# bupt-cist/vqa-playground-pytorch

Measured on AMD Instinct MI355X. Metric: VQA samples/sec (fwd+bwd), CoR2 batch 512, 36x2048 regions, higher is better.
Workload: dtype f32

## Files before the change

### vqa_playground_pytorch_amd/csrc/attention_logits.hip

```cpp
#include <cstdlib>
#include <type_traits>

#include "gemm_f32_rt.hpp"

namespace vqa {

constexpr int kAlMaxG = 8;
constexpr int kAlThreads = 256;
constexpr int kAlWaves = kAlThreads / 64;

template <typename T>
struct AlVec;
template <>
struct AlVec<float> {
  static constexpr int VEC = 2, P = 4;
  static __device__ __forceinline__ void ldb(rt::rsrc_t r, uint32_t voff, uint32_t soff, float (&v)[2]) {
    const auto t = __builtin_bit_cast(float2, __builtin_amdgcn_raw_buffer_load_b64(r, (int)voff, (int)soff, 0));
    v[0] = t.x;
    v[1] = t.y;
  }
  static __device__ __forceinline__ void stb(rt::rsrc_t r, uint32_t voff, uint32_t soff, const float (&v)[2]) {
    typedef unsigned int u32x2 __attribute__((ext_vector_type(2)));
    __builtin_amdgcn_raw_buffer_store_b64(u32x2{__float_as_uint(v[0]), __float_as_uint(v[1])}, r, (int)voff, (int)soff, 0);
  }
  static __device__ __forceinline__ void ld(const float* p, float (&v)[2]) {
    const float2 t = ld2(p);
    v[0] = t.x;
    v[1] = t.y;
  }
  static __device__ __forceinline__ void st(float* p, const float (&v)[2]) { st2(p, make_float2(v[0], v[1])); }
};
template <>
struct AlVec<bf16> {
  static constexpr int VEC = 4, P = 2;
  static __device__ __forceinline__ void ldb(rt::rsrc_t r, uint32_t voff, uint32_t soff, float (&v)[4]) {
    const auto w = __builtin_bit_cast(uint2, __builtin_amdgcn_raw_buffer_load_b64(r, (int)voff, (int)soff, 0));
    v[0] = bf16_lo(w.x);
    v[1] = bf16_hi(w.x);
    v[2] = bf16_lo(w.y);
    v[3] = bf16_hi(w.y);
  }
  static __device__ __forceinline__ void stb(rt::rsrc_t r, uint32_t voff, uint32_t soff, const float (&v)[4]) {
    typedef unsigned int u32x2 __attribute__((ext_vector_type(2)));
    __builtin_amdgcn_raw_buffer_store_b64(u32x2{pack_bf16(v[0], v[1]), pack_bf16(v[2], v[3])}, r, (int)voff, (int)soff, 0);
  }
  static __device__ __forceinline__ void ld(const bf16* p, float (&v)[4]) {
    const float4 t = ld4(p);
    v[0] = t.x;
    v[1] = t.y;
    v[2] = t.z;
    v[3] = t.w;
  }
  static __device__ __forceinline__ void st(bf16* p, const float (&v)[4]) { st4(p, make_float4(v[0], v[1], v[2], v[3])); }
};

struct AlMask {
  uint32_t key, p8;
  float scale;
};
__device__ __forceinline__ AlMask al_mask(const DropCfg& dc) { return AlMask{dc.p8 > 0 ? drop_key(dc) : 0u, dc.p8, dc.scale}; }
template <int MODE, int VEC>
__device__ __forceinline__ void al_keep(uint32_t e, const AlMask& mk, float (&s)[VEC]) {
#pragma unroll
  for (int j = 0; j < VEC; j += 2) {
    if constexpr (MODE == 0) {
      s[j] = 1.f, s[j + 1] = 1.f;
    } else if constexpr (MODE == 1) {
      const uint32_t w = mask_word32((e + j) >> 5, mk.key) >> ((e + j) & 31u);
      s[j] = (w & 1u) != 0u ? 2.f : 0.f;
      s[j + 1] = (w & 2u) != 0u ? 2.f : 0.f;
    } else {
      const uint32_t w = mask_word32((e + j) >> 2, mk.key) >> (8 * ((e + j) & 3));
      s[j] = (w & 255u) >= mk.p8 ? mk.scale : 0.f;
      s[j + 1] = ((w >> 8) & 255u) >= mk.p8 ? mk.scale : 0.f;
    }
  }
}
template <int G, int P, int VEC>
__device__ __forceinline__ void al_load_weights(const float* __restrict__ w, int K, int lane, float (&wr)[G][P][VEC]) {
#pragma unroll
  for (int g = 0; g < G; ++g)
#pragma unroll
    for (int p = 0; p < P; ++p)
#pragma unroll
      for (int j = 0; j < VEC; ++j) {
        const int k = (p * 64 + lane) * VEC + j;
        const float t = w[(size_t)g * K + min(k, K - 1)];
        wr[g][p][j] = k < K ? t : 0.f;
      }
}

constexpr int kAlRows = 8;

template <typename T, int G, int MODE>
__global__ __launch_bounds__(kAlThreads, 2) void attention_logits_fwd_kernel(const T* __restrict__ x, int ldx,
                                                                          const float* __restrict__ w,
                                                                          const float* __restrict__ bias,
                                                                          float* __restrict__ logits, int M, int K,
                                                                          DropCfg dc) {
  using V = AlVec<T>;
  constexpr int VEC = V::VEC, P = V::P, RB = kAlRows;
  constexpr bool BUTTERFLY = (RB * G) % 16 == 0 && 16 % G == 0;
  const int lane = threadIdx.x & 63;
  const int wave = blockIdx.x * kAlWaves + __builtin_amdgcn_readfirstlane(threadIdx.x >> 6), nwaves = gridDim.x * kAlWaves;
  float xv[RB][P][VEC];
  const int m_first = wave * RB;
  const rt::rsrc_t Xb = rt::make_rsrc(x, (size_t)M * ldx * sizeof(T));
  uint32_t voff[P];
#pragma unroll
  for (int p = 0; p < P; ++p) voff[p] = (uint32_t)min((p * 64 + lane) * VEC, ldx - VEC) * (uint32_t)sizeof(T);
  auto load_rows = [&](int m0) {
#pragma unroll
    for (int r = 0; r < RB; ++r) {
      const uint32_t soff = (uint32_t)min(m0 + r, M - 1) * (uint32_t)ldx * (uint32_t)sizeof(T);
#pragma unroll
      for (int p = 0; p < P; ++p) V::ldb(Xb, voff[p], soff, xv[r][p]);
    }
  };
  if (m_first < M) load_rows(m_first);
  float wr[G][P][VEC];
  al_load_weights<G, P, VEC>(w, K, lane, wr);
  const float bias_l = bias[(lane & 15) % G];
  const AlMask mk = al_mask(dc);
  for (int m0 = m_first; m0 < M; m0 += nwaves * RB) {
    if (m0 != m_first) load_rows(m0);
    float acc[RB][G];
    {
#pragma unroll
      for (int r = 0; r < RB; ++r) {
        const int m = min(m0 + r, M - 1);
#pragma unroll
        for (int g = 0; g < G; ++g) acc[r][g] = 0.f;
#pragma unroll
        for (int p = 0; p < P; ++p) {
          const int k = (p * 64 + lane) * VEC;
          float s[VEC];
          al_keep<MODE, VEC>((uint32_t)m * (uint32_t)K + (uint32_t)k, mk, s);
#pragma unroll
          for (int j = 0; j < VEC; ++j) {
            const float xs = xv[r][p][j] * s[j];
#pragma unroll
            for (int g = 0; g < G; ++g) acc[r][g] = fmaf(wr[g][p][j], xs, acc[r][g]);
          }
        }
        __builtin_amdgcn_sched_barrier(0);
      }
    }
    if constexpr (BUTTERFLY) {
      constexpr int RPB = 16 / G;
#pragma unroll
      for (int q = 0; q < RB / RPB; ++q) {
        float val[16];
#pragma unroll
        for (int i = 0; i < 16; ++i) val[i] = acc[q * RPB + i / G][i % G];
        const float t = rows_sum(row_reduce_scatter16(val, lane));
        const int m = m0 + q * RPB + (lane & 15) / G;
        if (lane < 16 && m < M) logits[(size_t)m * G + (lane & 15) % G] = t + bias_l;
      }
    } else {
#pragma unroll
      for (int r = 0; r < RB; ++r)
#pragma unroll
        for (int g = 0; g < G; ++g) {
          const float t = wave_sum(acc[r][g]);
          if (lane == 0 && m0 + r < M) logits[(size_t)(m0 + r) * G + g] = t + bias[g];
        }
    }
  }
}

constexpr int kAlBwdRows = 6;

template <typename T, int G, int MODE>
__global__ __launch_bounds__(kAlThreads, 2) void attention_logits_bwd_kernel(const T* __restrict__ x, int ldx,
                                                                          const float* __restrict__ w,
                                                                          const float* __restrict__ d_logits,
                                                                          T* __restrict__ d_x, float* __restrict__ part,
                                                                          float* __restrict__ partb, int M, int K,
                                                                          DropCfg dc) {
  using V = AlVec<T>;
  constexpr int VEC = V::VEC, P = V::P, RB = kAlBwdRows, KPAD = 64 * VEC * P;
  __shared__ float red_s[kAlWaves - 1][G][KPAD];
  __shared__ float redb_s[kAlWaves][G];
  const int lane = threadIdx.x & 63, wv = __builtin_amdgcn_readfirstlane(threadIdx.x >> 6);
  const int wave = blockIdx.x * kAlWaves + wv, nwaves = gridDim.x * kAlWaves;
  float wr[G][P][VEC], dw[G][P][VEC], db[G];
  al_load_weights<G, P, VEC>(w, K, lane, wr);
#pragma unroll
  for (int g = 0; g < G; ++g) {
    db[g] = 0.f;
#pragma unroll
    for (int p = 0; p < P; ++p)
#pragma unroll
      for (int j = 0; j < VEC; ++j) dw[g][p][j] = 0.f;
  }
  const AlMask mk = al_mask(dc);
  const rt::rsrc_t Xb = rt::make_rsrc(x, (size_t)M * ldx * sizeof(T));
  const rt::rsrc_t Db = rt::make_rsrc(d_x != nullptr ? d_x : const_cast<T*>(x), (size_t)M * ldx * sizeof(T));
  uint32_t voff[P];
#pragma unroll
  for (int p = 0; p < P; ++p) voff[p] = (uint32_t)min((p * 64 + lane) * VEC, ldx - VEC) * (uint32_t)sizeof(T);
  for (int m0 = wave * RB; m0 < M; m0 += nwaves * RB) {
    float xv[RB][P][VEC];
#pragma unroll
    for (int r = 0; r < RB; ++r) {
      const uint32_t soff = (uint32_t)min(m0 + r, M - 1) * (uint32_t)ldx * (uint32_t)sizeof(T);
#pragma unroll
      for (int p = 0; p < P; ++p) V::ldb(Xb, voff[p], soff, xv[r][p]);
    }
    float dl[RB][G];
#pragma unroll
    for (int r = 0; r < RB; ++r)
#pragma unroll
      for (int g = 0; g < G; ++g) {
        const float t = d_logits[(size_t)min(m0 + r, M - 1) * G + g];
        dl[r][g] = m0 + r < M ? t : 0.f;
      }
    {
#pragma unroll
      for (int r = 0; r < RB; ++r) {
        const int m = m0 + r;
#pragma unroll
        for (int g = 0; g < G; ++g) db[g] += dl[r][g];
#pragma unroll
        for (int p = 0; p < P; ++p) {
          const int k = (p * 64 + lane) * VEC;
          float s[VEC], o[VEC];
          al_keep<MODE, VEC>((uint32_t)min(m, M - 1) * (uint32_t)K + (uint32_t)k, mk, s);
#pragma unroll
          for (int j = 0; j < VEC; ++j) {
            const float xs = xv[r][p][j] * s[j];
            float t = 0.f;
#pragma unroll
            for (int g = 0; g < G; ++g) {
              dw[g][p][j] = fmaf(dl[r][g], xs, dw[g][p][j]);
              t = fmaf(dl[r][g], wr[g][p][j], t);
            }
            o[j] = t * s[j];
          }
          if (d_x != nullptr && m < M && k < ldx)
            V::stb(Db, (uint32_t)k * (uint32_t)sizeof(T), (uint32_t)m * (uint32_t)ldx * (uint32_t)sizeof(T), o);
        }
        __builtin_amdgcn_sched_barrier(0);
      }
    }
  }
  if (wv > 0) {
#pragma unroll
    for (int g = 0; g < G; ++g)
#pragma unroll
      for (int p = 0; p < P; ++p)
#pragma unroll
        for (int j = 0; j < VEC; ++j) red_s[wv - 1][g][(p * 64 + lane) * VEC + j] = dw[g][p][j];
  }
  if (lane == 0) {
#pragma unroll
    for (int g = 0; g < G; ++g) redb_s[wv][g] = db[g];
  }
  __syncthreads();
  if (wv == 0) {
#pragma unroll
    for (int g = 0; g < G; ++g)
#pragma unroll
      for (int p = 0; p < P; ++p)
#pragma unroll
        for (int j = 0; j < VEC; ++j) {
          const int k = (p * 64 + lane) * VEC + j;
          float t = dw[g][p][j];
#pragma unroll
          for (int q = 0; q < kAlWaves - 1; ++q) t += red_s[q][g][k];
          part[((size_t)blockIdx.x * G + g) * KPAD + k] = t;
        }
    if (lane < G) partb[(size_t)blockIdx.x * G + lane] = redb_s[0][lane] + redb_s[1][lane] + redb_s[2][lane] + redb_s[3][lane];
  }
}

__global__ __launch_bounds__(256) void attention_logits_finish_kernel(const float* __restrict__ part,
                                                                      const float* __restrict__ partb,
                                                                      float* __restrict__ d_w, float* __restrict__ d_bias,
                                                                      int K, int G, int KPAD, int nblocks) {
  __shared__ float red_s[16][17];
  const int c = threadIdx.x & 15, slice = threadIdx.x >> 4;
  const int e = blockIdx.x * 16 + c;
  const bool is_w = e < G * K, is_b = !is_w && e < G * K + G;
  const float* src = partb;
  size_t stride = (size_t)G, off = 0;
  if (is_w) {
    src = part;
    stride = (size_t)G * KPAD;
    off = (size_t)(e / K) * KPAD + (e % K);
  } else if (is_b) {
    off = (size_t)(e - G * K);
  }
  float a = 0.f;
  if (is_w || is_b) {
    for (int b0 = slice; b0 < nblocks; b0 += 256) {
      float t[16];
#pragma unroll
      for (int i = 0; i < 16; ++i) {
        const int b = b0 + 16 * i;
        t[i] = b < nblocks ? src[(size_t)b * stride + off] : 0.f;
      }
#pragma unroll
      for (int i = 0; i < 16; ++i) a += t[i];
    }
  }
  red_s[slice][c] = a;
  __syncthreads();
  if (slice == 0) {
    float t = 0.f;
#pragma unroll
    for (int q = 0; q < 16; ++q) t += red_s[q][c];
    if (is_w) d_w[e] = t;
    if (is_b) d_bias[e - G * K] = t;
  }
}

static int al_blocks(int M) {
  int b = (M + kAlBwdRows * kAlWaves - 1) / (kAlBwdRows * kAlWaves);
  if (b > 512) b = 512;
  if (b < 1) b = 1;
  return b;
}

template <typename T>
static int al_check(const char* who, const T* x, int ldx, int M, int K, int G, float p_drop) {
  using V = AlVec<T>;
  VQA_REQUIRE(M > 0 && K > 0 && G > 0, VQA_E_BADARG, "%s: bad sizes M=%d K=%d G=%d", who, M, K, G);
  VQA_REQUIRE(p_drop >= 0.f && p_drop < 1.f, VQA_E_BADARG, "%s: p_drop=%f outside [0,1)", who, (double)p_drop);
  VQA_REQUIRE(G <= kAlMaxG && K <= 64 * V::VEC * V::P && K % 2 == 0 && ldx >= K && ldx % V::VEC == 0 &&
                  aligned(x, V::VEC * sizeof(T)) && (size_t)M * ldx * sizeof(T) < (1ull << 32),
              VQA_E_UNSUPPORTED, "%s: needs G <= 8, even K <= %d, ldx %% %d == 0, aligned x, M*ldx*sizeof < 4 GiB (K=%d ldx=%d G=%d)", who,
              64 * V::VEC * V::P, V::VEC, K, ldx, G);
  return VQA_OK;
}

#define VQA_AL_SWITCH_G(G, CALL)      \
  switch (G) {                        \
    case 1: { CALL(1); } break;       \
    case 2: { CALL(2); } break;       \
    case 3: { CALL(3); } break;       \
    case 4: { CALL(4); } break;       \
    case 5: { CALL(5); } break;       \
    case 6: { CALL(6); } break;       \
    case 7: { CALL(7); } break;       \
    default: { CALL(8); } break;      \
  }

template <typename T>
static int al_fwd_impl(const char* who, const T* x, int ldx, const float* w, const float* bias, float* logits, float p_drop,
                       uint64_t seed, const uint64_t* seed_ptr, int M, int K, int G, vqa_stream_t stream) {
  VQA_REQUIRE(x && w && bias && logits, VQA_E_BADARG, "%s: null pointer", who);
  int rc = al_check(who, x, ldx, M, K, G, p_drop);
  if (rc != VQA_OK) return rc;
  hipStream_t s = static_cast<hipStream_t>(stream);
  const DropCfg dc = make_drop(p_drop, seed, seed_ptr);
  int blocks = (M + kAlRows * kAlWaves - 1) / (kAlRows * kAlWaves);
  if (blocks > 2048) blocks = 2048;
  const int mode = dc.p8 == 0 ? 0 : (dc.p8 == kDropHalf ? 1 : 2);
#define CALL_M(G_, MODE_) \
  VQA_LAUNCH((attention_logits_fwd_kernel<T, G_, MODE_>), dim3(blocks), dim3(kAlThreads), 0, s, x, ldx, w, bias, logits, M, K, dc)
#define CALL(G_)                       \
  if (mode == 0) CALL_M(G_, 0);        \
  else if (mode == 1) CALL_M(G_, 1);   \
  else CALL_M(G_, 2)
  VQA_AL_SWITCH_G(G, CALL);
#undef CALL
#undef CALL_M
  return check_launch(who);
}

template <typename T>
static size_t al_ws_bytes(int M, int G) {
  using V = AlVec<T>;
  return (size_t)al_blocks(M) * G * (64 * V::VEC * V::P + 1) * sizeof(float);
}

template <typename T>
static int al_bwd_impl(const char* who, const T* x, int ldx, const float* w, const float* d_logits, T* d_x, float* d_w,
                       float* d_bias, void* workspace, size_t workspace_bytes, float p_drop, uint64_t seed,
                       const uint64_t* seed_ptr, int M, int K, int G, vqa_stream_t stream) {
  using V = AlVec<T>;
  VQA_REQUIRE(x && w && d_logits && d_w && d_bias && workspace, VQA_E_BADARG, "%s: null pointer", who);
  int rc = al_check(who, x, ldx, M, K, G, p_drop);
  if (rc != VQA_OK) return rc;
  VQA_REQUIRE(d_x == nullptr || aligned(d_x, V::VEC * sizeof(T)), VQA_E_UNSUPPORTED, "%s: d_x is not aligned", who);
  VQA_REQUIRE(workspace_bytes >= al_ws_bytes<T>(M, G), VQA_E_BADARG, "%s: workspace of %zu B is too small", who, workspace_bytes);
  hipStream_t s = static_cast<hipStream_t>(stream);
  const DropCfg dc = make_drop(p_drop, seed, seed_ptr);
  const int blocks = al_blocks(M);
  constexpr int KPAD = 64 * V::VEC * V::P;
  float* part = static_cast<float*>(workspace);
  float* partb = part + (size_t)blocks * G * KPAD;
  const int mode = dc.p8 == 0 ? 0 : (dc.p8 == kDropHalf ? 1 : 2);
#define CALL_M(G_, MODE_)                                                                                                        \
  VQA_LAUNCH((attention_logits_bwd_kernel<T, G_, MODE_>), dim3(blocks), dim3(kAlThreads), 0, s, x, ldx, w, d_logits, d_x, \
                     part, partb, M, K, dc)
#define CALL(G_)                       \
  if (mode == 0) CALL_M(G_, 0);        \
  else if (mode == 1) CALL_M(G_, 1);   \
  else CALL_M(G_, 2)
  VQA_AL_SWITCH_G(G, CALL);
#undef CALL
#undef CALL_M
  VQA_LAUNCH(attention_logits_finish_kernel, dim3((G * K + G + 15) / 16), dim3(256), 0, s, part, partb, d_w, d_bias, K,
                     G, KPAD, blocks);
  return check_launch(who);
}

}

using namespace vqa;

extern "C" int vqa_attention_logits_fwd(const float* x, int ldx, const float* w, const float* bias, float* logits,
                                        float p_drop, uint64_t seed, const uint64_t* seed_ptr, int M, int K, int G,
                                        vqa_stream_t stream) {
  return al_fwd_impl<float>("attention_logits_fwd", x, ldx, w, bias, logits, p_drop, seed, seed_ptr, M, K, G, stream);
}
extern "C" int vqa_attention_logits_fwd_bf16(const vqa_bf16_t* x, int ldx, const float* w, const float* bias, float* logits,
                                             float p_drop, uint64_t seed, const uint64_t* seed_ptr, int M, int K, int G,
                                             vqa_stream_t stream) {
  return al_fwd_impl<bf16>("attention_logits_fwd_bf16", reinterpret_cast<const bf16*>(x), ldx, w, bias, logits, p_drop, seed,
                           seed_ptr, M, K, G, stream);
}
extern "C" size_t vqa_attention_logits_bwd_workspace_bytes(int M, int K, int G) {
  if (M <= 0 || K <= 0 || G <= 0 || G > kAlMaxG) return 0;
  return al_ws_bytes<float>(M, G) > al_ws_bytes<bf16>(M, G) ? al_ws_bytes<float>(M, G) : al_ws_bytes<bf16>(M, G);
}
extern "C" int vqa_attention_logits_bwd(const float* x, int ldx, const float* w, const float* d_logits, float* d_x,
                                        float* d_w, float* d_bias, void* workspace, size_t workspace_bytes, float p_drop,
                                        uint64_t seed, const uint64_t* seed_ptr, int M, int K, int G, vqa_stream_t stream) {
  return al_bwd_impl<float>("attention_logits_bwd", x, ldx, w, d_logits, d_x, d_w, d_bias, workspace, workspace_bytes, p_drop,
                            seed, seed_ptr, M, K, G, stream);
}
extern "C" int vqa_attention_logits_bwd_bf16(const vqa_bf16_t* x, int ldx, const float* w, const float* d_logits,
                                             vqa_bf16_t* d_x, float* d_w, float* d_bias, void* workspace,
                                             size_t workspace_bytes, float p_drop, uint64_t seed, const uint64_t* seed_ptr,
                                             int M, int K, int G, vqa_stream_t stream) {
  return al_bwd_impl<bf16>("attention_logits_bwd_bf16", reinterpret_cast<const bf16*>(x), ldx, w, d_logits,
                           reinterpret_cast<bf16*>(d_x), d_w, d_bias, workspace, workspace_bytes, p_drop, seed, seed_ptr, M, K,
                           G, stream);
}
```

Measured before the change: 260,800.

## Triple-buffer row loads and widen vector accesses in attention logits kernels

Result: no change. 261,200, median of 4 (+0.2%).

```diff
diff --git a/vqa_playground_pytorch_amd/csrc/attention_logits.hip b/vqa_playground_pytorch_amd/csrc/attention_logits.hip
--- a/vqa_playground_pytorch_amd/csrc/attention_logits.hip
+++ b/vqa_playground_pytorch_amd/csrc/attention_logits.hip
@@ -6,91 +6,106 @@
 namespace vqa {
 
 constexpr int kAlMaxG = 8;
-constexpr int kAlThreads = 256;
-constexpr int kAlWaves = kAlThreads / 64;
+constexpr int kAlCus = 256;
+constexpr int kAlKpad = 512;
+constexpr int kAlThreads = 256, kAlWaves = kAlThreads / 64;
+constexpr int kAlBwdThreads = 512, kAlBwdWaves = kAlBwdThreads / 64;
+static_assert(kAlBwdThreads == kAlKpad, "the backward kernel's LDS pass gives every thread one column");
 
 template <typename T>
 struct AlVec;
 template <>
 struct AlVec<float> {
-  static constexpr int VEC = 2, P = 4;
-  static __device__ __forceinline__ void ldb(rt::rsrc_t r, uint32_t voff, uint32_t soff, float (&v)[2]) {
-    const auto t = __builtin_bit_cast(float2, __builtin_amdgcn_raw_buffer_load_b64(r, (int)voff, (int)soff, 0));
-    v[0] = t.x;
-    v[1] = t.y;
-  }
-  static __device__ __forceinline__ void stb(rt::rsrc_t r, uint32_t voff, uint32_t soff, const float (&v)[2]) {
-    typedef unsigned int u32x2 __attribute__((ext_vector_type(2)));
-    __builtin_amdgcn_raw_buffer_store_b64(u32x2{__float_as_uint(v[0]), __float_as_uint(v[1])}, r, (int)voff, (int)soff, 0);
-  }
-  static __device__ __forceinline__ void ld(const float* p, float (&v)[2]) {
-    const float2 t = ld2(p);
-    v[0] = t.x;
-    v[1] = t.y;
-  }
-  static __device__ __forceinline__ void st(float* p, const float (&v)[2]) { st2(p, make_float2(v[0], v[1])); }
+  static constexpr int VEC = 4, P = 2, HALF = 2;
+  static __device__ __forceinline__ void unpack(rt::u32x4 r, float (&v)[4]) {
+#pragma unroll
+    for (int j = 0; j < 4; ++j) v[j] = __uint_as_float(r[j]);
+  }
+  static __device__ __forceinline__ rt::u32x4 pack(const float (&v)[4]) {
+    return rt::u32x4{__float_as_uint(v[0]), __float_as_uint(v[1]), __float_as_uint(v[2]), __float_as_uint(v[3])};
+  }
 };
 template <>
 struct AlVec<bf16> {
-  static constexpr int VEC = 4, P = 2;
-  static __device__ __forceinline__ void ldb(rt::rsrc_t r, uint32_t voff, uint32_t soff, float (&v)[4]) {
-    const auto w = __builtin_bit_cast(uint2, __builtin_amdgcn_raw_buffer_load_b64(r, (int)voff, (int)soff, 0));
-    v[0] = bf16_lo(w.x);
-    v[1] = bf16_hi(w.x);
-    v[2] = bf16_lo(w.y);
-    v[3] = bf16_hi(w.y);
-  }
-  static __device__ __forceinline__ void stb(rt::rsrc_t r, uint32_t voff, uint32_t soff, const float (&v)[4]) {
-    typedef unsigned int u32x2 __attribute__((ext_vector_type(2)));
-    __builtin_amdgcn_raw_buffer_store_b64(u32x2{pack_bf16(v[0], v[1]), pack_bf16(v[2], v[3])}, r, (int)voff, (int)soff, 0);
-  }
-  static __device__ __forceinline__ void ld(const bf16* p, float (&v)[4]) {
-    const float4 t = ld4(p);
-    v[0] = t.x;
-    v[1] = t.y;
-    v[2] = t.z;
-    v[3] = t.w;
-  }
-  static __device__ __forceinline__ void st(bf16* p, const float (&v)[4]) { st4(p, make_float4(v[0], v[1], v[2], v[3])); }
+  static constexpr int VEC = 8, P = 1, HALF = 4;
+  static __device__ __forceinline__ void unpack(rt::u32x4 r, float (&v)[8]) {
+#pragma unroll
+    for (int j = 0; j < 4; ++j) v[2 * j] = bf16_lo(r[j]), v[2 * j + 1] = bf16_hi(r[j]);
+  }
+  static __device__ __forceinline__ rt::u32x4 pack(const float (&v)[8]) {
+    return rt::u32x4{pack_bf16(v[0], v[1]), pack_bf16(v[2], v[3]), pack_bf16(v[4], v[5]), pack_bf16(v[6], v[7])};
+  }
 };
+__device__ __forceinline__ rt::u32x4 al_ldb(rt::rsrc_t r, uint32_t voff, uint32_t soff) {
+  return __builtin_amdgcn_raw_buffer_load_b128(r, (int)voff, (int)soff, 0);
+}
+__device__ __forceinline__ void al_stb(rt::rsrc_t r, uint32_t voff, uint32_t soff, rt::u32x4 v) {
+  __builtin_amdgcn_raw_buffer_store_b128(v, r, (int)voff, (int)soff, 0);
+}
+__device__ __forceinline__ void al_stb_half(rt::rsrc_t r, uint32_t voff, uint32_t soff, rt::u32x4 v) {
+  typedef unsigned int u32x2 __attribute__((ext_vector_type(2)));
+  __builtin_amdgcn_raw_buffer_store_b64(u32x2{v[0], v[1]}, r, (int)voff, (int)soff, 0);
+}
 
 struct AlMask {
   uint32_t key, p8;
   float scale;
 };
 __device__ __forceinline__ AlMask al_mask(const DropCfg& dc) { return AlMask{dc.p8 > 0 ? drop_key(dc) : 0u, dc.p8, dc.scale}; }
+template <int MODE>
+__device__ __forceinline__ uint32_t al_row_words(uint32_t e_row, int lane, const AlMask& mk) {
+  if constexpr (MODE == 1) return mask_word32((e_row >> 5) + (uint32_t)lane, mk.key);
+  return 0u;
+}
 template <int MODE, int VEC>
-__device__ __forceinline__ void al_keep(uint32_t e, const AlMask& mk, float (&s)[VEC]) {
-#pragma unroll
-  for (int j = 0; j < VEC; j += 2) {
-    if constexpr (MODE == 0) {
-      s[j] = 1.f, s[j + 1] = 1.f;
-    } else if constexpr (MODE == 1) {
-      const uint32_t w = mask_word32((e + j) >> 5, mk.key) >> ((e + j) & 31u);
-      s[j] = (w & 1u) != 0u ? 2.f : 0.f;
-      s[j + 1] = (w & 2u) != 0u ? 2.f : 0.f;
-    } else {
-      const uint32_t w = mask_word32((e + j) >> 2, mk.key) >> (8 * ((e + j) & 3));
-      s[j] = (w & 255u) >= mk.p8 ? mk.scale : 0.f;
-      s[j + 1] = ((w >> 8) & 255u) >= mk.p8 ? mk.scale : 0.f;
+__device__ __forceinline__ void al_keep(uint32_t e_row, uint32_t col, uint32_t row_words, const AlMask& mk, float (&s)[VEC]) {
+  if constexpr (MODE == 0) {
+#pragma unroll
+    for (int j = 0; j < VEC; ++j) s[j] = 1.f;
+  } else if constexpr (MODE == 1) {
+    const uint32_t bp = (e_row & 31u) + col;
+    const int at = (int)((bp >> 5) << 2);
+    const uint32_t w0 = (uint32_t)__builtin_amdgcn_ds_bpermute(at, (int)row_words);
+    const uint32_t w1 = (uint32_t)__builtin_amdgcn_ds_bpermute(at + 4, (int)row_words);
+    const uint32_t bits = __builtin_amdgcn_alignbit(w1, w0, bp & 31u);
+#pragma unroll
+    for (int j = 0; j < VEC; ++j) s[j] = __uint_as_float((0u - ((bits >> j) & 1u)) & 0x40000000u);
+  } else {
+    const uint32_t wi = (e_row + col) >> 2, shift = 8u * (e_row & 3u);
+    uint32_t hw[VEC / 4 + 1];
+#pragma unroll
+    for (int i = 0; i < VEC / 4; ++i) hw[i] = mask_word32(wi + (uint32_t)i, mk.key);
+    hw[VEC / 4] = shift != 0u ? mask_word32(wi + (uint32_t)(VEC / 4), mk.key) : 0u;
+#pragma unroll
+    for (int i = 0; i < VEC / 4; ++i) {
+      const uint32_t v = __builtin_amdgcn_alignbit(hw[i + 1], hw[i], shift);
+#pragma unroll
+      for (int b = 0; b < 4; ++b) s[4 * i + b] = ((v >> (8 * b)) & 255u) >= mk.p8 ? mk.scale : 0.f;
     }
   }
 }
 template <int G, int P, int VEC>
 __device__ __forceinline__ void al_load_weights(const float* __restrict__ w, int K, int lane, float (&wr)[G][P][VEC]) {
+  const rt::rsrc_t Wb = rt::make_rsrc(w, (size_t)G * K * sizeof(float));
 #pragma unroll
   for (int g = 0; g < G; ++g)
 #pragma unroll
     for (int p = 0; p < P; ++p)
 #pragma unroll
-      for (int j = 0; j < VEC; ++j) {
+      for (int j = 0; j < VEC; j += 4) {
         const int k = (p * 64 + lane) * VEC + j;
-        const float t = w[(size_t)g * K + min(k, K - 1)];
-        wr[g][p][j] = k < K ? t : 0.f;
+        const rt::u32x4 t = al_ldb(Wb, (uint32_t)k * (uint32_t)sizeof(float), (uint32_t)(g * K) * (uint32_t)sizeof(float));
+#pragma unroll
+        for (int i = 0; i < 4; ++i) wr[g][p][j + i] = k + i < K ? __uint_as_float(t[i]) : 0.f;
       }
 }
 
-constexpr int kAlRows = 8;
+constexpr int kAlRows = 3;
+
+__device__ __forceinline__ void al_share(int wave, int nwaves, int M, int& lo, int& hi) {
+  lo = (int)((long long)wave * M / nwaves);
+  hi = (int)((long long)(wave + 1) * M / nwaves);
+}
 
 template <typename T, int G, int MODE>
 __global__ __launch_bounds__(kAlThreads, 2) void attention_logits_fwd_kernel(const T* __restrict__ x, int ldx,
@@ -100,62 +115,66 @@
                                                                           DropCfg dc) {
   using V = AlVec<T>;
   constexpr int VEC = V::VEC, P = V::P, RB = kAlRows;
-  constexpr bool BUTTERFLY = (RB * G) % 16 == 0 && 16 % G == 0;
+  constexpr bool BUTTERFLY = 16 % G == 0;
   const int lane = threadIdx.x & 63;
   const int wave = blockIdx.x * kAlWaves + __builtin_amdgcn_readfirstlane(threadIdx.x >> 6), nwaves = gridDim.x * kAlWaves;
-  float xv[RB][P][VEC];
-  const int m_first = wave * RB;
+  int m_lo, m_hi;
+  al_share(wave, nwaves, M, m_lo, m_hi);
+  if (m_lo >= m_hi) return;
   const rt::rsrc_t Xb = rt::make_rsrc(x, (size_t)M * ldx * sizeof(T));
-  uint32_t voff[P];
-#pragma unroll
-  for (int p = 0; p < P; ++p) voff[p] = (uint32_t)min((p * 64 + lane) * VEC, ldx - VEC) * (uint32_t)sizeof(T);
-  auto load_rows = [&](int m0) {
+  uint32_t col[P];
+#pragma unroll
+  for (int p = 0; p < P; ++p) col[p] = (uint32_t)((p * 64 + lane) * VEC);
+  auto load_rows = [&](rt::u32x4 (&buf)[RB][P], int m0) {
 #pragma unroll
     for (int r = 0; r < RB; ++r) {
-      const uint32_t soff = (uint32_t)min(m0 + r, M - 1) * (uint32_t)ldx * (uint32_t)sizeof(T);
-#pragma unroll
-      for (int p = 0; p < P; ++p) V::ldb(Xb, voff[p], soff, xv[r][p]);
+      const uint32_t soff = (uint32_t)min(m0 + r, m_hi - 1) * (uint32_t)ldx * (uint32_t)sizeof(T);
+#pragma unroll
+      for (int p = 0; p < P; ++p) buf[r][p] = al_ldb(Xb, col[p] * (uint32_t)sizeof(T), soff);
     }
   };
-  if (m_first < M) load_rows(m_first);
+  rt::u32x4 b0[RB][P], b1[RB][P], b2[RB][P];
+  load_rows(b0, m_lo);
+  load_rows(b1, m_lo + RB);
   float wr[G][P][VEC];
   al_load_weights<G, P, VEC>(w, K, lane, wr);
   const float bias_l = bias[(lane & 15) % G];
   const AlMask mk = al_mask(dc);
-  for (int m0 = m_first; m0 < M; m0 += nwaves * RB) {
-    if (m0 != m_first) load_rows(m0);
+  auto work = [&](const rt::u32x4 (&buf)[RB][P], int m0) {
     float acc[RB][G];
-    {
-#pragma unroll
-      for (int r = 0; r < RB; ++r) {
-        const int m = min(m0 + r, M - 1);
-#pragma unroll
-        for (int g = 0; g < G; ++g) acc[r][g] = 0.f;
+#pragma unroll
+    for (int r = 0; r < RB; ++r) {
+#pragma unroll
+      for (int g = 0; g < G; ++g) acc[r][g] = 0.f;
+      if (m0 + r < m_hi) {
+        const uint32_t e_row = (uint32_t)(m0 + r) * (uint32_t)K;
+        const uint32_t words = al_row_words<MODE>(e_row, lane, mk);
 #pragma unroll
         for (int p = 0; p < P; ++p) {
-          const int k = (p * 64 + lane) * VEC;
-          float s[VEC];
-          al_keep<MODE, VEC>((uint32_t)m * (uint32_t)K + (uint32_t)k, mk, s);
+          float xv[VEC], s[VEC];
+          V::unpack(buf[r][p], xv);
+          al_keep<MODE, VEC>(e_row, col[p], words, mk, s);
 #pragma unroll
           for (int j = 0; j < VEC; ++j) {
-            const float xs = xv[r][p][j] * s[j];
+            const float xk = (int)col[p] + j < K ? xv[j] : 0.f;
+            const float xs = MODE == 0 ? xk : xk * s[j];
 #pragma unroll
             for (int g = 0; g < G; ++g) acc[r][g] = fmaf(wr[g][p][j], xs, acc[r][g]);
           }
         }
-        __builtin_amdgcn_sched_barrier(0);
       }
+      __builtin_amdgcn_sched_barrier(0);
     }
     if constexpr (BUTTERFLY) {
       constexpr int RPB = 16 / G;
 #pragma unroll
-      for (int q = 0; q < RB / RPB; ++q) {
+      for (int q = 0; q * RPB < RB; ++q) {
         float val[16];
 #pragma unroll
-        for (int i = 0; i < 16; ++i) val[i] = acc[q * RPB + i / G][i % G];
+        for (int i = 0; i < 16; ++i) val[i] = q * RPB + i / G < RB ? acc[min(q * RPB + i / G, RB - 1)][i % G] : 0.f;
         const float t = rows_sum(row_reduce_scatter16(val, lane));
-        const int m = m0 + q * RPB + (lane & 15) / G;
-        if (lane < 16 && m < M) logits[(size_t)m * G + (lane & 15) % G] = t + bias_l;
+        const int r = q * RPB + (lane & 15) / G;
+        if (lane < 16 && r < RB && m0 + r < m_hi) logits[(size_t)(m0 + r) * G + (lane & 15) % G] = t + bias_l;
       }
     } else {
 #pragma unroll
@@ -163,115 +182,148 @@
 #pragma unroll
         for (int g = 0; g < G; ++g) {
           const float t = wave_sum(acc[r][g]);
-          if (lane == 0 && m0 + r < M) logits[(size_t)(m0 + r) * G + g] = t + bias[g];
+          if (lane == 0 && m0 + r < m_hi) logits[(size_t)(m0 + r) * G + g] = t + bias[g];
         }
     }
-  }
-}
-
-constexpr int kAlBwdRows = 6;
+  };
+  for (int m0 = m_lo;; m0 += 3 * RB) {
+    load_rows(b2, m0 + 2 * RB);
+    work(b0, m0);
+    if (m0 + RB >= m_hi) break;
+    load_rows(b0, m0 + 3 * RB);
+    work(b1, m0 + RB);
+    if (m0 + 2 * RB >= m_hi) break;
+    load_rows(b1, m0 + 4 * RB);
+    work(b2, m0 + 2 * RB);
+    if (m0 + 3 * RB >= m_hi) break;
+  }
+}
 
 template <typename T, int G, int MODE>
-__global__ __launch_bounds__(kAlThreads, 2) void attention_logits_bwd_kernel(const T* __restrict__ x, int ldx,
-                                                                          const float* __restrict__ w,
-                                                                          const float* __restrict__ d_logits,
-                                                                          T* __restrict__ d_x, float* __restrict__ part,
-                                                                          float* __restrict__ partb, int M, int K,
-                                                                          DropCfg dc) {
+__global__ __launch_bounds__(kAlBwdThreads, 2) void attention_logits_bwd_kernel(const T* __restrict__ x, int ldx,
+                                                                             const float* __restrict__ w,
+                                                                             const float* __restrict__ d_logits,
+                                                                             T* __restrict__ d_x, float* __restrict__ part,
+                                                                             float* __restrict__ partb, int M, int K,
+                                                                             DropCfg dc) {
   using V = AlVec<T>;
-  constexpr int VEC = V::VEC, P = V::P, RB = kAlBwdRows, KPAD = 64 * VEC * P;
-  __shared__ float red_s[kAlWaves - 1][G][KPAD];
-  __shared__ float redb_s[kAlWaves][G];
+  constexpr int VEC = V::VEC, P = V::P, RB = kAlRows, NW = kAlBwdWaves;
+  __shared__ __attribute__((aligned(16))) float red_s[2][NW][kAlKpad];
+  __shared__ float redb_s[NW][RB * G];
   const int lane = threadIdx.x & 63, wv = __builtin_amdgcn_readfirstlane(threadIdx.x >> 6);
-  const int wave = blockIdx.x * kAlWaves + wv, nwaves = gridDim.x * kAlWaves;
-  float wr[G][P][VEC], dw[G][P][VEC], db[G];
-  al_load_weights<G, P, VEC>(w, K, lane, wr);
-#pragma unroll
-  for (int g = 0; g < G; ++g) {
-    db[g] = 0.f;
-#pragma unroll
-    for (int p = 0; p < P; ++p)
-#pragma unroll
-      for (int j = 0; j < VEC; ++j) dw[g][p][j] = 0.f;
-  }
-  const AlMask mk = al_mask(dc);
+  const int wave = blockIdx.x * NW + wv, nwaves = gridDim.x * NW;
+  int m_lo, m_hi;
+  al_share(wave, nwaves, M, m_lo, m_hi);
   const rt::rsrc_t Xb = rt::make_rsrc(x, (size_t)M * ldx * sizeof(T));
   const rt::rsrc_t Db = rt::make_rsrc(d_x != nullptr ? d_x : const_cast<T*>(x), (size_t)M * ldx * sizeof(T));
-  uint32_t voff[P];
-#pragma unroll
-  for (int p = 0; p < P; ++p) voff[p] = (uint32_t)min((p * 64 + lane) * VEC, ldx - VEC) * (uint32_t)sizeof(T);
-  for (int m0 = wave * RB; m0 < M; m0 += nwaves * RB) {
-    float xv[RB][P][VEC];
+  const rt::rsrc_t Lb = rt::make_rsrc(d_logits, (size_t)M * G * sizeof(float));
+  uint32_t col[P];
+  bool st_full[P], st_half[P];
+#pragma unroll
+  for (int p = 0; p < P; ++p) {
+    col[p] = (uint32_t)((p * 64 + lane) * VEC);
+    st_full[p] = (int)col[p] + VEC <= ldx;
+    st_half[p] = !st_full[p] && (int)col[p] < ldx;
+  }
+  const uint32_t lcol = (uint32_t)min(lane, RB * G - 1) * (uint32_t)sizeof(float);
+  auto load_rows = [&](rt::u32x4 (&buf)[RB][P], float& dlv, int m0) {
 #pragma unroll
     for (int r = 0; r < RB; ++r) {
-      const uint32_t soff = (uint32_t)min(m0 + r, M - 1) * (uint32_t)ldx * (uint32_t)sizeof(T);
-#pragma unroll
-      for (int p = 0; p < P; ++p) V::ldb(Xb, voff[p], soff, xv[r][p]);
-    }
-    float dl[RB][G];
-#pragma unroll
-    for (int r = 0; r < RB; ++r)
-#pragma unroll
-      for (int g = 0; g < G; ++g) {
-        const float t = d_logits[(size_t)min(m0 + r, M - 1) * G + g];
-        dl[r][g] = m0 + r < M ? t : 0.f;
+      const uint32_t soff = (uint32_t)min(m0 + r, m_hi - 1) * (uint32_t)ldx * (uint32_t)sizeof(T);
+#pragma unroll
+      for (int p = 0; p < P; ++p) buf[r][p] = al_ldb(Xb, col[p] * (uint32_t)sizeof(T), soff);
+    }
+    dlv = rt::ldg4(Lb, lcol, (uint32_t)__builtin_amdgcn_readfirstlane(m0 * (int)(G * sizeof(float))));
+  };
+  rt::u32x4 b0[RB][P], b1[RB][P], b2[RB][P];
+  float dl0 = 0.f, dl1 = 0.f, dl2 = 0.f;
+  if (m_lo < m_hi) {
+    load_rows(b0, dl0, m_lo);
+    load_rows(b1, dl1, m_lo + RB);
+  }
+  float wr[G][P][VEC], dw[G][P][VEC], dbv = 0.f;
+  al_load_weights<G, P, VEC>(w, K, lane, wr);
+#pragma unroll
+  for (int g = 0; g < G; ++g)
+#pragma unroll
+    for (int p = 0; p < P; ++p)
+#pragma unroll
+      for (int j = 0; j < VEC; ++j) dw[g][p][j] = 0.f;
+  const AlMask mk = al_mask(dc);
+  auto work = [&](const rt::u32x4 (&buf)[RB][P], float dlv, int m0) {
+    dlv = lane < RB * G && m0 + lane / G < m_hi ? dlv : 0.f;
+    dbv += dlv;
+#pragma unroll
+    for (int r = 0; r < RB; ++r) {
+      if (m0 + r < m_hi) {
+        const int m = m0 + r;
+        float dl[G];
+#pragma unroll
+        for (int g = 0; g < G; ++g) dl[g] = __int_as_float(__builtin_amdgcn_readlane(__float_as_int(dlv), r * G + g));
+        const uint32_t e_row = (uint32_t)m * (uint32_t)K;
+        const uint32_t words = al_row_words<MODE>(e_row, lane, mk);
+        const uint32_t soff = (uint32_t)m * (uint32_t)ldx * (uint32_t)sizeof(T);
+#pragma unroll
+        for (int p = 0; p < P; ++p) {
+          float xv[VEC], s[VEC], o[VEC];
+          V::unpack(buf[r][p], xv);
+          al_keep<MODE, VEC>(e_row, col[p], words, mk, s);
+#pragma unroll
+          for (int j = 0; j < VEC; ++j) {
+            const float xk = (int)col[p] + j < K ? xv[j] : 0.f;
+            const float xs = MODE == 0 ? xk : xk * s[j];
+            float t = 0.f;
+#pragma unroll
+            for (int g = 0; g < G; ++g) {
+              dw[g][p][j] = fmaf(dl[g], xs, dw[g][p][j]);
+              t = fmaf(dl[g], wr[g][p][j], t);
+            }
+            o[j] = MODE == 0 ? t : t * s[j];
+          }
+          if (d_x != nullptr) {
+            const rt::u32x4 ov = V::pack(o);
+            if (st_full[p]) al_stb(Db, col[p] * (uint32_t)sizeof(T), soff, ov);
+            if (st_half[p]) al_stb_half(Db, col[p] * (uint32_t)sizeof(T), soff, ov);
+          }
+        }
       }
-    {
-#pragma unroll
-      for (int r = 0; r < RB; ++r) {
-        const int m = m0 + r;
-#pragma unroll
-        for (int g = 0; g < G; ++g) db[g] += dl[r][g];
-#pragma unroll
-        for (int p = 0; p < P; ++p) {
-          const int k = (p * 64 + lane) * VEC;
-          float s[VEC], o[VEC];
-          al_keep<MODE, VEC>((uint32_t)min(m, M - 1) * (uint32_t)K + (uint32_t)k, mk, s);
-#pragma unroll
-          for (int j = 0; j < VEC; ++j) {
-            const float xs = xv[r][p][j] * s[j];
-            float t = 0.f;
-#pragma unroll
-            for (int g = 0; g < G; ++g) {
-              dw[g][p][j] = fmaf(dl[r][g], xs, dw[g][p][j]);
-              t = fmaf(dl[r][g], wr[g][p][j], t);
-            }
-            o[j] = t * s[j];
-          }
-          if (d_x != nullptr && m < M && k < ldx)
-            V::stb(Db, (uint32_t)k * (uint32_t)sizeof(T), (uint32_t)m * (uint32_t)ldx * (uint32_t)sizeof(T), o);
-        }
-        __builtin_amdgcn_sched_barrier(0);
-      }
-    }
-  }
-  if (wv > 0) {
-#pragma unroll
-    for (int g = 0; g < G; ++g)
-#pragma unroll
-      for (int p = 0; p < P; ++p)
-#pragma unroll
-        for (int j = 0; j < VEC; ++j) red_s[wv - 1][g][(p * 64 + lane) * VEC + j] = dw[g][p][j];
-  }
-  if (lane == 0) {
-#pragma unroll
-    for (int g = 0; g < G; ++g) redb_s[wv][g] = db[g];
-  }
-  __syncthreads();
-  if (wv == 0) {
-#pragma unroll
-    for (int g = 0; g < G; ++g)
-#pragma unroll
-      for (int p = 0; p < P; ++p)
-#pragma unroll
-        for (int j = 0; j < VEC; ++j) {
-          const int k = (p * 64 + lane) * VEC + j;
-          float t = dw[g][p][j];
-#pragma unroll
-          for (int q = 0; q < kAlWaves - 1; ++q) t += red_s[q][g][k];
-          part[((size_t)blockIdx.x * G + g) * KPAD + k] = t;
-        }
-    if (lane < G) partb[(size_t)blockIdx.x * G + lane] = redb_s[0][lane] + redb_s[1][lane] + redb_s[2][lane] + redb_s[3][lane];
+      __builtin_amdgcn_sched_barrier(0);
+    }
+  };
+  if (m_lo < m_hi) {
+    for (int m0 = m_lo;; m0 += 3 * RB) {
+      load_rows(b2, dl2, m0 + 2 * RB);
+      work(b0, dl0, m0);
+      if (m0 + RB >= m_hi) break;
+      load_rows(b0, dl0, m0 + 3 * RB);
+      work(b1, dl1, m0 + RB);
+      if (m0 + 2 * RB >= m_hi) break;
+      load_rows(b1, dl1, m0 + 4 * RB);
+      work(b2, dl2, m0 + 2 * RB);
+      if (m0 + 3 * RB >= m_hi) break;
+    }
+  }
+  if (lane < RB * G) redb_s[wv][lane] = dbv;
+#pragma unroll
+  for (int g = 0; g < G; ++g) {
+#pragma unroll
+    for (int p = 0; p < P; ++p)
+#pragma unroll
+      for (int j = 0; j < VEC; j += 4)
+        st4(&red_s[g & 1][wv][col[p] + j], make_float4(dw[g][p][j], dw[g][p][j + 1], dw[g][p][j + 2], dw[g][p][j + 3]));
+    __syncthreads();
+    float t = red_s[g & 1][0][threadIdx.x];
+#pragma unroll
+    for (int q = 1; q < NW; ++q) t += red_s[g & 1][q][threadIdx.x];
+    part[((size_t)blockIdx.x * G + g) * kAlKpad + threadIdx.x] = t;
+  }
+  if (threadIdx.x < G) {
+    float t = 0.f;
+#pragma unroll
+    for (int q = 0; q < NW; ++q)
+#pragma unroll
+      for (int r = 0; r < RB; ++r) t += redb_s[q][r * G + threadIdx.x];
+    partb[(size_t)blockIdx.x * G + threadIdx.x] = t;
   }
 }
 
@@ -316,22 +368,22 @@
   }
 }
 
-static int al_blocks(int M) {
-  int b = (M + kAlBwdRows * kAlWaves - 1) / (kAlBwdRows * kAlWaves);
-  if (b > 512) b = 512;
-  if (b < 1) b = 1;
-  return b;
-}
+static int al_blocks(int M, int waves, int per_cu) {
+  const int b = (M + kAlRows * waves - 1) / (kAlRows * waves);
+  return b < 1 ? 1 : (b > per_cu * kAlCus ? per_cu * kAlCus : b);
+}
+static int al_fwd_blocks(int M) { return al_blocks(M, kAlWaves, 2); }
+static int al_bwd_blocks(int M) { return al_blocks(M, kAlBwdWaves, 1); }
 
 template <typename T>
 static int al_check(const char* who, const T* x, int ldx, int M, int K, int G, float p_drop) {
   using V = AlVec<T>;
   VQA_REQUIRE(M > 0 && K > 0 && G > 0, VQA_E_BADARG, "%s: bad sizes M=%d K=%d G=%d", who, M, K, G);
   VQA_REQUIRE(p_drop >= 0.f && p_drop < 1.f, VQA_E_BADARG, "%s: p_drop=%f outside [0,1)", who, (double)p_drop);
-  VQA_REQUIRE(G <= kAlMaxG && K <= 64 * V::VEC * V::P && K % 2 == 0 && ldx >= K && ldx % V::VEC == 0 &&
-                  aligned(x, V::VEC * sizeof(T)) && (size_t)M * ldx * sizeof(T) < (1ull << 32),
+  VQA_REQUIRE(G <= kAlMaxG && K <= kAlKpad && K % 2 == 0 && ldx >= K && ldx % V::HALF == 0 &&
+                  aligned(x, V::HALF * sizeof(T)) && (size_t)M * ldx * sizeof(T) < (1ull << 32),
               VQA_E_UNSUPPORTED, "%s: needs G <= 8, even K <= %d, ldx %% %d == 0, aligned x, M*ldx*sizeof < 4 GiB (K=%d ldx=%d G=%d)", who,
-              64 * V::VEC * V::P, V::VEC, K, ldx, G);
+              kAlKpad, V::HALF, K, ldx, G);
   return VQA_OK;
 }
 
@@ -355,8 +407,7 @@
   if (rc != VQA_OK) return rc;
   hipStream_t s = static_cast<hipStream_t>(stream);
   const DropCfg dc = make_drop(p_drop, seed, seed_ptr);
-  int blocks = (M + kAlRows * kAlWaves - 1) / (kAlRows * kAlWaves);
-  if (blocks > 2048) blocks = 2048;
+  const int blocks = al_fwd_blocks(M);
   const int mode = dc.p8 == 0 ? 0 : (dc.p8 == kDropHalf ? 1 : 2);
 #define CALL_M(G_, MODE_) \
   VQA_LAUNCH((attention_logits_fwd_kernel<T, G_, MODE_>), dim3(blocks), dim3(kAlThreads), 0, s, x, ldx, w, bias, logits, M, K, dc)
@@ -370,11 +421,7 @@
   return check_launch(who);
 }
 
-template <typename T>
-static size_t al_ws_bytes(int M, int G) {
-  using V = AlVec<T>;
-  return (size_t)al_blocks(M) * G * (64 * V::VEC * V::P + 1) * sizeof(float);
-}
+static size_t al_ws_bytes(int M, int G) { return (size_t)al_bwd_blocks(M) * G * (kAlKpad + 1) * sizeof(float); }
 
 template <typename T>
 static int al_bwd_impl(const char* who, const T* x, int ldx, const float* w, const float* d_logits, T* d_x, float* d_w,
@@ -384,17 +431,18 @@
   VQA_REQUIRE(x && w && d_logits && d_w && d_bias && workspace, VQA_E_BADARG, "%s: null pointer", who);
   int rc = al_check(who, x, ldx, M, K, G, p_drop);
   if (rc != VQA_OK) return rc;
-  VQA_REQUIRE(d_x == nullptr || aligned(d_x, V::VEC * sizeof(T)), VQA_E_UNSUPPORTED, "%s: d_x is not aligned", who);
-  VQA_REQUIRE(workspace_bytes >= al_ws_bytes<T>(M, G), VQA_E_BADARG, "%s: workspace of %zu B is too small", who, workspace_bytes);
+  VQA_REQUIRE(d_x == nullptr || aligned(d_x, V::HALF * sizeof(T)), VQA_E_UNSUPPORTED, "%s: d_x is not aligned", who);
+  VQA_REQUIRE((size_t)M * G * sizeof(float) < (1ull << 32), VQA_E_UNSUPPORTED, "%s: needs M*G*4 < 4 GiB (M=%d G=%d)", who, M, G);
+  VQA_REQUIRE(workspace_bytes >= al_ws_bytes(M, G), VQA_E_BADARG, "%s: workspace of %zu B is too small", who, workspace_bytes);
   hipStream_t s = static_cast<hipStream_t>(stream);
   const DropCfg dc = make_drop(p_drop, seed, seed_ptr);
-  const int blocks = al_blocks(M);
-  constexpr int KPAD = 64 * V::VEC * V::P;
+  const int blocks = al_bwd_blocks(M);
+  constexpr int KPAD = kAlKpad;
   float* part = static_cast<float*>(workspace);
   float* partb = part + (size_t)blocks * G * KPAD;
   const int mode = dc.p8 == 0 ? 0 : (dc.p8 == kDropHalf ? 1 : 2);
 #define CALL_M(G_, MODE_)                                                                                                        \
-  VQA_LAUNCH((attention_logits_bwd_kernel<T, G_, MODE_>), dim3(blocks), dim3(kAlThreads), 0, s, x, ldx, w, d_logits, d_x, \
+  VQA_LAUNCH((attention_logits_bwd_kernel<T, G_, MODE_>), dim3(blocks), dim3(kAlBwdThreads), 0, s, x, ldx, w, d_logits, d_x, \
                      part, partb, M, K, dc)
 #define CALL(G_)                       \
   if (mode == 0) CALL_M(G_, 0);        \
@@ -425,7 +473,7 @@
 }
 extern "C" size_t vqa_attention_logits_bwd_workspace_bytes(int M, int K, int G) {
   if (M <= 0 || K <= 0 || G <= 0 || G > kAlMaxG) return 0;
-  return al_ws_bytes<float>(M, G) > al_ws_bytes<bf16>(M, G) ? al_ws_bytes<float>(M, G) : al_ws_bytes<bf16>(M, G);
+  return al_ws_bytes(M, G);
 }
 extern "C" int vqa_attention_logits_bwd(const float* x, int ldx, const float* w, const float* d_logits, float* d_x,
                                         float* d_w, float* d_bias, void* workspace, size_t workspace_bytes, float p_drop,
```
